# yfukasawa/LongQC

Measured on AMD Instinct MI355X. Metric: Mbases/sec all-vs-all overlap coverage (sampleqc hot path), higher is better.
Workload: dtype u64; 1 GPU; BASELINE configs[2]: 500000 synthetic PacBio Sequel CLR reads ~10 kb 30x, pb-sequel preset (-Y -l 0 -q 160 -k 12 -w 5 -I 4G -p 80), 5000 subsample queries; target_bases=5181693140, query_bases=51577117, parallelism=single GPU

## Files before the change

### longqc_amd/csrc/engine.cpp

```cpp
#include "engine.hpp"
#include "kernels_sketch.hpp"
#include "kernels_index.hpp"
#include "kernels_seed.hpp"
#include "kernels_sort.hpp"
#include "kernels_walk.hpp"
#include "kernels_psort.hpp"
#include "kernels_chain.hpp"
#include "fastx.hpp"
#include "fastx_mem.hpp"
#include "sat_replay.hpp"
#ifndef LQ_EMU
extern "C" void lq_segv_altstack();
#endif
#include <cstdio>
#include <cstring>
#include <cmath>
#include <cinttypes>
#include <algorithm>
#include <unordered_map>
#include <deque>
#include <future>
#include <functional>

static inline u32 nblk(u64 n, u32 bs)
{
	u64 b = (n + bs - 1) / bs;
	if (b > 0x7fffffffULL) throw std::runtime_error("launch too large");
	return (u32)b;
}

template <class T> static void h2d(T *dst, const T *src, size_t n, hipStream_t s)
{
	if (n) LQ_HIP_CHECK(hipMemcpyAsync(dst, src, n * sizeof(T), hipMemcpyHostToDevice, s));
}
template <class T> static void d2h(T *dst, const T *src, size_t n, hipStream_t s)
{
	if (n) { LQ_HIP_CHECK(hipMemcpyAsync(dst, src, n * sizeof(T), hipMemcpyDeviceToHost, s)); LQ_HIP_CHECK(hipStreamSynchronize(s)); }
}
static void dzero(void *p, size_t bytes, hipStream_t s) { if (bytes) LQ_HIP_CHECK(hipMemsetAsync(p, 0, bytes, s)); }
static void check_launch() { LQ_HIP_CHECK(hipGetLastError()); }
static const bool lq_timeline = getenv("LQCOV_TIMELINE") != nullptr;
static double lq_timeline_t0 = 0;
static void lq_tl(const char *who, int id, const char *what, double extra = -1)
{
	if (!lq_timeline) return;
	if (extra >= 0) fprintf(stderr, "[tl] %8.2f %s%d %s %.0f\n", (lq_now_s() - lq_timeline_t0) * 1e3, who, id, what, extra);
	else fprintf(stderr, "[tl] %8.2f %s%d %s\n", (lq_now_s() - lq_timeline_t0) * 1e3, who, id, what);
}
#ifndef LQ_EMU
int lq_trace_launches = 0;
#endif

StageTimer::StageTimer(lqcov_handle *h_, hipStream_t s_, const char *name_, u64 bytes_) : h(h_), s(s_), name(name_), bytes(bytes_)
{
	on = h->profiling && (h->profile_only.empty() || h->profile_only == name_ || ("|" + h->profile_only + "|").find(std::string("|") + name_ + "|") != std::string::npos);
	if (!on) return;
	hipEventCreate(&a); hipEventCreate(&b);
	hipEventRecord(a, s);
}
StageTimer::StageTimer(lqcov_handle *h_, const char *name_, u64 bytes_) : StageTimer(h_, h_->stream, name_, bytes_) {}
StageTimer::~StageTimer()
{
	if (!on) return;
	hipEventRecord(b, s);
	if (h->profiling == 1) { hipEventSynchronize(b); std::lock_guard<std::mutex> g(h->stage_mu); h->account_stage(name, a, b, bytes); }
	else { std::lock_guard<std::mutex> g(h->stage_mu); h->stage_pending.push_back(lqcov_handle::StagePending{name, a, b, bytes}); }
}
void lqcov_handle::account_stage(const char *name, hipEvent_t a, hipEvent_t b, u64 bytes)
{
	float ms = 0; hipEventElapsedTime(&ms, a, b);
	hipEventDestroy(a); hipEventDestroy(b);
	auto it = stages.find(name);
	if (it == stages.end()) { stage_order.push_back(name); it = stages.emplace(name, StageAcc()).first; }
	it->second.ms += ms; it->second.launches += 1; it->second.bytes += bytes;
}
void lqcov_handle::drain_stages()
{
	std::lock_guard<std::mutex> g(stage_mu);
	for (lqcov_handle::StagePending &sp : stage_pending) { hipEventSynchronize(sp.b); account_stage(sp.name, sp.a, sp.b, sp.bytes); }
	stage_pending.clear();
	for (auto &kv : late_bytes) { auto it = stages.find(kv.first); if (it != stages.end()) it->second.bytes += kv.second; }
	late_bytes.clear();
}
void lqcov_handle::add_stage_bytes(const char *name, u64 bytes)
{
	if (!profiling || !bytes) return;
	std::lock_guard<std::mutex> g(stage_mu);
	late_bytes[name] += bytes;
}

void Knobs::read_env()
{
	auto num = [](const char *name, long dflt) { const char *e = getenv(name); return e && *e ? atol(e) : dflt; };
	auto is = [](const char *name, const char *val) { const char *e = getenv(name); return e && !strcmp(e, val); };
	lanes = (int)std::min<long>(8, std::max<long>(1, num("LQCOV_LANES", 3)));
	anchor_budget = getenv("LQCOV_ANCHOR_BUDGET") ? strtoull(getenv("LQCOV_ANCHOR_BUDGET"), 0, 10) : 0;
	query_order_file = is("LQCOV_QUERY_ORDER", "file");
	query_order_striped = is("LQCOV_QUERY_ORDER", "striped");
	all_klib = is("LQCOV_SORT", "klib");
	ps_shift = (u32)std::min<long>(12, std::max<long>(0, num("LQCOV_PS_SHIFT", 0)));
	reg_walker = !is("LQCOV_WALK", "solo");
	ckpt = !is("LQCOV_CKPT", "0");
	ckpt3 = num("LQCOV_CKPT3", 1) > 0;
	sort_tile = (u32)std::max<long>(0, num("LQCOV_SORT_TILE", 0)); if (sort_tile && sort_tile < 64) sort_tile = 64;
	walk_shift = (u32)std::min<long>(16, std::max<long>(0, num("LQCOV_WALK_SHIFT", 0)));
	chain_wave_min = (int)std::max<long>(0, num("LQCOV_CHAIN_WAVE_MIN", 0));
	chain_cap = (int)num("LQCOV_CHAIN_CAP", 128);
	run_stage = (u32)std::max<long>(1, num("LQCOV_RUN_STAGE", LQ_RUN_STAGE));
	run_grid = (u32)std::max<long>(1, num("LQCOV_RUN_GRID", 2048));
	ps_key64 = num("LQCOV_PS_KEY64", 0) != 0;
	sketch_wgen = num("LQCOV_SKETCH_WGEN", 0) != 0;
	upload_amb = num("LQCOV_UPLOAD_AMB", 0) != 0;
	sketch_fast = num("LQCOV_SKETCH_FAST", 1) != 0;
#ifndef LQ_EMU
	lq_trace_launches = (int)num("LQCOV_TRACE_LAUNCHES", 0);
#endif
	no_level_skip = getenv("LQCOV_NO_LEVEL_SKIP") != nullptr;
	debug_sort = getenv("LQCOV_DEBUG_SORT") != nullptr;
	sketch_kpt = (u32)std::min<long>(64, std::max<long>(1, num("LQCOV_SKETCH_KPT", 4)));
	sketch_machine_only = is("LQCOV_SKETCH", "machine");
// ... 568 lines not shown
{
	const u32 n = q.n;
	dzero(lambda.p, (n + 1) * 8, stream); dzero(lambda2.p, (n + 1) * 8, stream);
	dzero(avg_k.p, (n + 1) * 4, stream); dzero(qflags.p, (n + 1) * 4, stream);
	dzero(cnts.p, cnt_count() * 4 + 4, stream);
	dzero(n_pv.p, 4, stream);
	if (!distributed) mid_occ = -1;
	stat_sens_runs = 0; stat_p2_queries = 0; stat_p2_anchors = 0;
	for (auto &v : stat_tie_why) v = 0;
	sat_cnt.clear(); stat_sat_chains = 0; sat_last_valid = false;
	finished = false;
	LQ_HIP_CHECK(hipStreamSynchronize(stream));
	if (lq_timeline) { lq_timeline_t0 = lq_now_s(); lq_tl("main", 0, "reset"); }
}

void lqcov_handle::build_index(Part &pt)
{
	hipStream_t stream = this->bstream; Prim &prim = this->bprim;
	(void)prim;
	ReadSetDev &rs = pt.rs;
	const u64 M = rs.n_mini;
	ix_owner = &pt;
	sat_last_valid = false;
	pt.n_keys = 0; pt.cap_bits = 4;
	pt.pos.ensure(M * 8 + 8);
	std::vector<u32> soff(q.n + 1, 0), srid;
	bool names_done = false;
	auto host_names = [&]() {
		names_done = true;
		if (P.no_self && q.n) {
			std::unordered_map<std::string, std::vector<u32>> byname;
			for (u32 i = 0; i < q.n; ++i) byname[q.names[i]].push_back(i);
			std::vector<std::vector<u32>> per(q.n);
			for (u32 r = 0; r < rs.n; ++r) {
				auto it = byname.find(rs.names[r]);
				if (it != byname.end()) for (u32 qi : it->second) per[qi].push_back(r);
			}
			for (u32 i = 0; i < q.n; ++i) { soff[i + 1] = soff[i] + (u32)per[i].size(); srid.insert(srid.end(), per[i].begin(), per[i].end()); }
		}
		if (P.ava) {
			std::vector<std::string> names(rs.names.begin(), rs.names.end());
			std::sort(names.begin(), names.end());
			names.erase(std::unique(names.begin(), names.end()), names.end());
			std::vector<u32> tr(rs.n + 1, 0), ql(q.n + 1, 0);
			for (u32 r = 0; r < rs.n; ++r) tr[r] = (u32)(std::lower_bound(names.begin(), names.end(), rs.names[r]) - names.begin());
			for (u32 i = 0; i < q.n; ++i) ql[i] = (u32)(std::lower_bound(names.begin(), names.end(), q.names[i]) - names.begin());
			pt.t_rank.ensure((rs.n + 1) * 4); pt.q_lo.ensure((q.n + 1) * 4);
			h2d(pt.t_rank.as<u32>(), tr.data(), rs.n + 1, stream);
			h2d(pt.q_lo.as<u32>(), ql.data(), q.n + 1, stream);
			LQ_HIP_CHECK(hipStreamSynchronize(stream));
		}
	};
	if (M) {
		DBuf &key = ix_key, &key2 = ix_key2, &head = ix_head, &uidx = ix_uidx, &ukey = ix_ukey, &ustart = ix_ustart, &ucnt = ix_ucnt;
		const u64 n_tiles = (M + LQ_HEAD_TILE - 1) / LQ_HEAD_TILE;
		key.ensure(M * 8); key2.ensure(M * 8); head.ensure((n_tiles + 1) * 4); uidx.ensure((n_tiles + 1) * 8);
		const bool k32 = 2 * P.k <= 32;
		const bool fused_heads = 2 * P.k <= 24;
		if (k32) {
			if (!(rs.key_stamp && rs.key_stamp == ix_key_stamp)) { LQ_LAUNCH(k_sort_keys<u32>, nblk(M, 256), 256, stream, rs.mx.as<u64>(), M, key.as<u32>()); check_launch(); }
			ix_key_stamp = 0;
			{ StageTimer t(this, stream, "index_radix_sort", M * 24); prim.sort_pairs_u32_u64(key.as<u32>(), key2.as<u32>(), rs.my.as<u64>(), pt.pos.as<u64>(), M, (unsigned)(2 * P.k), key.as<u32>()); }
			if (!fused_heads) { LQ_LAUNCH(k_head_count<u32>, (u32)n_tiles, LQ_HEAD_THREADS, stream, key2.as<u32>(), M, head.as<u32>()); check_launch(); }
		} else {
			ix_key_stamp = 0;
			LQ_LAUNCH(k_sort_keys<u64>, nblk(M, 256), 256, stream, rs.mx.as<u64>(), M, key.as<u64>()); check_launch();
			{ StageTimer t(this, stream, "index_radix_sort", M * 32); prim.sort_pairs_u64(key.as<u64>(), key2.as<u64>(), rs.my.as<u64>(), pt.pos.as<u64>(), M, (unsigned)(2 * P.k), key.as<u64>()); }
			LQ_LAUNCH(k_head_count<u64>, (u32)n_tiles, LQ_HEAD_THREADS, stream, key2.as<u64>(), M, head.as<u32>()); check_launch();
		}
		u64 K = 0;
		if (fused_heads) {
			const u64 k_max = std::min<u64>(M, (u64)1 << (2 * P.k));
			ukey.ensure(k_max * 8); ustart.ensure(k_max * 8);
			const u64 n_blocks = (n_tiles + LQ_HEADLB_SUB - 1) / LQ_HEADLB_SUB;
			uidx.ensure((n_blocks + 2) * 8 + 64);
			dzero(uidx.p, (n_blocks + 2) * 8 + 64, stream);
			u64 *granules = uidx.as<u64>(), *count = granules + n_blocks; u32 *ticket = (u32*)(granules + n_blocks + 1);
			{
				StageTimer t(this, stream, "k_head_lookback", M * 4);
				LQ_LAUNCH(k_head_lookback<u32>, (u32)n_blocks, LQ_HEAD_THREADS, stream, key2.as<u32>(), M, granules, ticket, ukey.as<u64>(), ustart.as<u64>(), count);
				check_launch();
			}
			host_names();
			d2h(&K, count, 1, stream);
			pt.n_keys = K;
			ucnt.ensure(K * 4);
		} else {
			dzero(head.as<u32>() + n_tiles, 4, stream);
			prim.exclusive_scan_u32_u64(head.as<u32>(), uidx.as<u64>(), n_tiles + 1);
			host_names();
			d2h(&K, uidx.as<u64>() + n_tiles, 1, stream);
			pt.n_keys = K;
			ukey.ensure(K * 8); ustart.ensure(K * 8); ucnt.ensure(K * 4);
			if (k32) LQ_LAUNCH(k_head_fill<u32>, (u32)n_tiles, LQ_HEAD_THREADS, stream, key2.as<u32>(), M, uidx.as<u64>(), ukey.as<u64>(), ustart.as<u64>());
			else LQ_LAUNCH(k_head_fill<u64>, (u32)n_tiles, LQ_HEAD_THREADS, stream, key2.as<u64>(), M, uidx.as<u64>(), ukey.as<u64>(), ustart.as<u64>());
			check_launch();
		}
		LQ_LAUNCH(k_unique_counts, nblk(K, 256), 256, stream, ustart.as<u64>(), K, M, ucnt.as<u32>()); check_launch();
		u32 bits = 4;
		while (((u64)1 << bits) < 2 * K) ++bits;
		pt.cap_bits = bits;
		const u64 cap = (u64)1 << bits;
		pt.tkey.ensure(cap * 8); pt.tstart.ensure(cap * 8); pt.tcnt.ensure(cap * 4);
		LQ_HIP_CHECK(hipMemsetAsync(pt.tkey.p, 0xff, cap * 8, stream));
		{
			StageTimer t(this, stream, "k_table_insert", K * 20 + cap * 8);
			LQ_LAUNCH(k_table_insert, nblk(K, 256), 256, stream, ukey.as<u64>(), ustart.as<u64>(), ucnt.as<u32>(), K, pt.tkey.as<u64>(), pt.tstart.as<u64>(), pt.tcnt.as<u32>(), bits);
			check_launch();
		}
		if (mid_occ <= 0) {
			if (P.mid_occ_frac <= 0.0f) mid_occ = INT32_MAX;
			else {
				DBuf &sorted = ix_sorted; sorted.ensure(K * 4);
				prim.sort_keys_u32(ucnt.as<u32>(), sorted.as<u32>(), K);
				const u32 kth = (u32)((1. - P.mid_occ_frac) * (double)K);
				u32 v = 0;
				d2h(&v, sorted.as<u32>() + kth, 1, stream);
				mid_occ = (i32)(v + 1);
			}
		}
		LQ_HIP_CHECK(hipStreamSynchronize(stream));
	} else {
		const u64 cap = (u64)1 << pt.cap_bits;
		pt.tkey.ensure(cap * 8); pt.tstart.ensure(cap * 8); pt.tcnt.ensure(cap * 4);
		LQ_HIP_CHECK(hipMemsetAsync(pt.tkey.p, 0xff, cap * 8, stream));
		if (mid_occ <= 0) mid_occ = P.mid_occ_frac <= 0.0f ? INT32_MAX : 1;
	}
	if (!names_done) host_names();
	pt.self_off.ensure((q.n + 1) * 4); pt.self_rid.ensure(srid.size() * 4 + 4);
	h2d(pt.self_off.as<u32>(), soff.data(), q.n + 1, stream);
	h2d(pt.self_rid.as<u32>(), srid.data(), srid.size(), stream);
	LQ_HIP_CHECK(hipStreamSynchronize(stream));
	pt.built = true;
	pt.plan.valid = false;
	lq_tl("build", 0, "index done");
	if (K.plan_ahead && have_queries && mid_occ > 0 && !distributed) plan_part(pt, stream, prim);
}

void lqcov_handle::build_part(Part &pt)
{
	if (!have_queries) throw std::logic_error("set the queries before building a part");
	lq_tl("build", 0, "build_part begins (reads uploaded)");
	sketch(pt.rs, true);
	lq_tl("build", 0, "sketched");
	build_index(pt);
	lq_tl("build", 0, "index + seed plan done");
}

static u64 dbg_anchor_sum(const mm128 &a) { u64 h = (a.x * 0x9E3779B97F4A7C15ULL) ^ (a.y * 0xD6E8FEB86659FD93ULL); return h ^ (h >> 29); }

void lqcov_handle::sort_checked(MapLane &L, Part &pt, const u64 *aqb, const u32 *qkb, u32 nqb, u64 a_base, u64 nA, const std::vector<u64> &h_off, const std::vector<u32> &h_klib)
{
	mm128 *dA = L.A.as<mm128>(), *dB = L.B.as<mm128>();
	u64 sum_before = 0;
	if (K.debug_sort) {
		std::vector<mm128> ha(nA), hb(nA);
		d2h(ha.data(), dA, nA, L.stream); d2h(hb.data(), dB, nA, L.stream);
		for (u32 q = 0; q < nqb; ++q)
			for (u64 i = h_off[q]; i < h_off[q + 1]; ++i) sum_before += dbg_anchor_sum(h_klib[q] ? hb[i] : ha[i]);
	}
	sort_batch(L, pt, aqb, qkb, nqb, a_base, nA);
	if (K.debug_sort) {
		std::vector<mm128> ha(nA);
		d2h(ha.data(), dA, nA, L.stream);
		u64 sum_after = 0;
		for (u64 i = 0; i < nA; ++i) sum_after += dbg_anchor_sum(ha[i]);
		if (sum_after != sum_before) fprintf(stderr, "[sort] batch of %u queries: NOT A PERMUTATION of the emitted anchors (sums %016llx / %016llx)\n", nqb, (unsigned long long)sum_before, (unsigned long long)sum_after);
		u64 unsorted = 0, ties = 0, unmarked = 0;
		for (u32 q = 0; q < nqb; ++q)
			for (u64 i = h_off[q] + 1; i < h_off[q + 1]; ++i) {
				if (ha[i].x < ha[i - 1].x) ++unsorted;
				if (ha[i].x == ha[i - 1].x) { ++ties; if (!(ha[i].y & LQ_TIE_MARK) || !(ha[i - 1].y & LQ_TIE_MARK)) { if (unmarked++ < 4) fprintf(stderr, "[sort] query %u of the batch: equal x %016llx, y %016llx / %016llx\n", q, (unsigned long long)ha[i].x, (unsigned long long)ha[i - 1].y, (unsigned long long)ha[i].y); } }
			}
		fprintf(stderr, "[sort] batch of %u queries: %llu anchors, %llu out of order, %llu equal-x neighbours, %llu of them with an unmarked anchor\n", nqb, (unsigned long long)nA, (unsigned long long)unsorted, (unsigned long long)ties, (unsigned long long)unmarked);
// ... 233 lines not shown
		}
	} else if (nj && opt) {
		StageTimer t(this, L.stream, "k_seed_emit", nj * 32 + nA * 24);
		LQ_LAUNCH(k_seed_emit, nblk(nj, LQ_EMIT_THREADS), LQ_EMIT_THREADS, L.stream, q.mx.as<u64>(), q.my.as<u64>(), q_owner.as<u32>(), q.moff.as<u64>(), j0, nj,
		          pt.pos.as<u64>(), hit_start.as<u64>(), hit_n.as<u32>(), keep.as<u32>(), dup.as<u32>(),
		          a_off.as<u64>(), a_base, mp_off.as<u64>(), q.d_len.as<u32>(),
		          (int)P.no_self, pt.self_off.as<u32>(), pt.self_rid.as<u32>(), ava,
		          qzero.as<u32>(), L.A.as<mm128>(), L.B.as<mm128>(), mini_pos.as<u64>(), EmitSub{nullptr, nullptr, nullptr});
		check_launch();
	}
	const u32 ivl_cap = (u32)std::min<u64>(nA / (P.min_cnt > 0 ? P.min_cnt : 1) + 16, 0xfffffff0ULL);
	L.ivl.ensure((u64)ivl_cap * sizeof(Ivl));
	dzero(L.n_ivl.p, 4, L.stream); dzero(L.n_sens.p, 32, L.stream);
	if (nA) {
		const u64 *aqb = (opt ? aqf_off : aq_off).as<u64>() + q0;
		const u32 *qkb = opt ? qzero.as<u32>() : qklib.as<u32>() + q0;
		std::vector<u64> rel; std::vector<u32> hk;
		if (K.debug_sort) {
			rel.resize(nqb + 1); hk.assign(nqb, 0);
			for (u32 i = 0; i <= nqb; ++i) rel[i] = h_off[q0 + i] - a_base;
			if (!opt) d2h(hk.data(), qklib.as<u32>() + q0, nqb, L.stream);
		}
		sort_checked(L, pt, aqb, qkb, nqb, a_base, nA, rel, hk);
		if (opt && !L.gate_passed) { L.gate_passed = true; open_gate(); }
		chain_stage(L, pt, aqb, a_base, nqb, q0, nullptr, nA, opt ? 1 : 0, 0, ivl_cap, dbg);
	}
	u32 n_sens = 0;
	if (nA && opt) {
		u32 ns8[8] = {0};
		d2h(ns8, L.n_sens.as<u32>(), 8, L.stream);
		n_sens = ns8[0];
		for (int i = 1; i <= 6; ++i) stat_tie_why[i - 1] += ns8[i];
	}
	lq_tl("lane", lane_id, "first pass done, anchors", (double)nA);
	if (n_sens) {
		std::vector<u64> want(n_sens);
		d2h(want.data(), L.sens.as<u64>(), n_sens, L.stream);
		std::sort(want.begin(), want.end());
		want.erase(std::unique(want.begin(), want.end()), want.end());
		std::vector<u32> fq;
		for (u64 k : want) if (fq.empty() || fq.back() != (u32)(k >> 32)) fq.push_back((u32)(k >> 32));
		L.want.ensure(want.size() * 8);
		h2d(L.want.as<u64>(), want.data(), want.size(), L.stream);
		LQ_HIP_CHECK(hipStreamSynchronize(L.stream));
		stat_sens_runs += want.size(); stat_p2_queries += fq.size();
		u64 max_mini = 0;
		for (size_t i = 0; i < fq.size(); ) {
			std::vector<u32> sq, sk; std::vector<u64> so{0};
			size_t k = i;
			while (k < fq.size() && (k == i || so.back() + (h_aq[fq[k] + 1] - h_aq[fq[k]]) <= anchor_budget)) {
				const u64 len = h_aq[fq[k] + 1] - h_aq[fq[k]];
				sq.push_back(fq[k]); sk.push_back(len > LQ_RS_MIN ? 1u : 0u); so.push_back(so.back() + len);
				max_mini = std::max<u64>(max_mini, h_qmoff[fq[k] + 1] - h_qmoff[fq[k]]);
				++k;
			}
			stat_p2_anchors += so.back();
			lq_tl("lane", lane_id, "second pass begins, anchors", (double)so.back());
			map_subset(L, pt, sq, sk, so, max_mini, 2, (u32)want.size(), ivl_cap, dbg, nullptr);
			if (lq_timeline) { LQ_HIP_CHECK(hipStreamSynchronize(L.stream)); lq_tl("lane", lane_id, "second pass done"); }
			i = k;
		}
	}
	if (nA) {
		u32 ni = 0;
		d2h(&ni, L.n_ivl.as<u32>(), 1, L.stream);
		if (ni > ivl_cap) throw std::runtime_error("interval pool overflow");
		if (ni) {
			L.iv_q.ensure((u64)ni * 4); L.iv_q2.ensure((u64)ni * 4); L.iv_se.ensure((u64)ni * 8); L.iv_se2.ensure((u64)ni * 8);
			L.ivq_off.ensure((n_q + 1) * 4); L.iv_scratch.ensure((u64)ni * 16);
			LQ_LAUNCH(k_split_ivl, nblk(ni, 256), 256, L.stream, L.ivl.as<Ivl>(), ni, L.iv_q.as<u32>(), L.iv_se.as<u64>()); check_launch();
			L.prim.sort_pairs_u32_u64(L.iv_q.as<u32>(), L.iv_q2.as<u32>(), L.iv_se.as<u64>(), L.iv_se2.as<u64>(), ni, 32);
			LQ_LAUNCH(k_ivl_offsets, nblk(n_q + 1, 256), 256, L.stream, L.iv_q2.as<u32>(), ni, n_q, L.ivq_off.as<u32>()); check_launch();
			std::lock_guard<std::mutex> guard(pv_mu);
			const u64 need = pv_reserved + 2 * (u64)ni;
			if (need > 0xfffffff0ULL) throw std::domain_error("too many persisted intervals");
			if (need > pv_cap) {
				LQ_HIP_CHECK(hipDeviceSynchronize());
				u32 npv = 0;
				d2h(&npv, n_pv.as<u32>(), 1, L.stream);
				grow_keep(pv, (u64)npv * sizeof(Ivl), need * sizeof(Ivl) * 2, L.stream);
				pv_cap = (u32)std::min<u64>(pv.cap / sizeof(Ivl), 0xfffffff0ULL);
			}
			pv_reserved = need;
			StageTimer t(this, L.stream, "k_filter_redundant");
			LQ_LAUNCH(k_filter_redundant, nblk(n_q, 64), 64, L.stream, L.iv_se2.as<u64>(), L.ivq_off.as<u32>(), n_q, (u32)P.min_coverage,
			          L.iv_scratch.as<u32>(), pv.as<Ivl>(), n_pv.as<u32>(), pv_cap);
			check_launch();
		}
	}
}

static PsLists ps_lists(MapLane &L, int set, u32 sh)
{
	PsWork &W = L.ps[set];
	PsLists Ls;
	Ls.big[0] = W.big[0].as<PSeg>(); Ls.big[1] = W.big[1].as<PSeg>(); Ls.fin_s = W.fin_s.as<PSeg>(); Ls.fin_b = W.fin_b.as<PSeg>();
	Ls.cnt = L.sort_cnt.as<u32>() + (set ? LQ_C_PS1 : LQ_C_PS0);
	Ls.cap_big = (u32)std::min<u64>(W.big[0].cap / sizeof(PSeg), 0xfffffff0ULL); Ls.cap_fin = (u32)std::min<u64>(W.fin_s.cap / sizeof(PSeg), 0xfffffff0ULL);
	Ls.fin_s_max = std::max<u32>(LQ_PS_FIN_SMALL >> sh, 2); Ls.fin_b_max = std::max<u32>(LQ_PS_FIN_BIG >> sh, 4); Ls.child_target = std::max<u32>(LQ_PS_CHILD >> sh, 2);
	return Ls;
}

static void ps_pass(lqcov_handle *h, MapLane &L, int set, hipStream_t s, u64 nA, const KeyMap &km, const PsData &pd, u32 cur)
{
	PsWork &W = L.ps[set];
	u32 *cnt = L.sort_cnt.as<u32>() + (set ? LQ_C_PS1 : LQ_C_PS0);
	const PsLists Ls = ps_lists(L, set, h->K.ps_shift);
	const u32 cap_cnt = (u32)std::min<u64>(W.gcnt.cap / 4, 0xfffffff0ULL);
	const u32 g_tiles = (u32)std::min<u64>((nA + LQ_PS_TILE - 1) / LQ_PS_TILE + 1, LQ_PS_GRID);
	const u32 g_segs = (u32)std::min<u64>(Ls.cap_big, 256);
	const u32 nxt = cur ^ 1;
	const u32 cap_tiles = (u32)std::min<u64>(W.tmap.cap / 4, 0xfffffff0ULL);
	LQ_LAUNCH(k_ps_plan, 1, 256, s, Ls.big[cur], cnt + (cur ? LQ_P_BIG1 : LQ_P_BIG0), W.plan.as<PPlan>(), cnt, cap_cnt, cap_tiles, Ls.child_target, cnt + (nxt ? LQ_P_BIG1 : LQ_P_BIG0)); check_launch();
	LQ_LAUNCH(k_ps_tilemap, g_segs, 256, s, W.plan.as<PPlan>(), cnt + (cur ? LQ_P_BIG1 : LQ_P_BIG0), cnt, W.tmap.as<u32>(), cap_tiles, W.gcnt.as<u32>(), W.gdiff.as<unsigned long long>()); check_launch();
	{
		StageTimer t(h, s, "k_ps_hist");
		LQ_LAUNCH(k_ps_hist, g_tiles, LQ_PS_THREADS, s, Ls.big[cur], cnt + (cur ? LQ_P_BIG1 : LQ_P_BIG0), W.plan.as<PPlan>(), W.tmap.as<u32>(), cnt, pd, km, W.gcnt.as<u32>(), W.gdiff.as<unsigned long long>()); check_launch();
	}
	LQ_LAUNCH(k_ps_scan, g_segs, 256, s, Ls.big[cur], cnt + (cur ? LQ_P_BIG1 : LQ_P_BIG0), W.plan.as<PPlan>(), W.gcnt.as<u32>(), W.gcur.as<u32>(), W.gdiff.as<unsigned long long>(), Ls, (u32)(nxt ? LQ_P_BIG1 : LQ_P_BIG0),
	          (unsigned long long*)(L.sort_cnt.as<u32>() + (set ? LQ_C_PART1 : LQ_C_PART0))); check_launch();
	{
		StageTimer t(h, s, "k_ps_scatter");
		LQ_LAUNCH(k_ps_scatter, g_tiles, LQ_PS_THREADS, s, Ls.big[cur], cnt + (cur ? LQ_P_BIG1 : LQ_P_BIG0), W.plan.as<PPlan>(), W.tmap.as<u32>(), cnt, pd, km, W.gcur.as<u32>()); check_launch();
	}
}

static void ps_finish(lqcov_handle *h, MapLane &L, int set, hipStream_t s, u64 nA, const KeyMap &km, const PsData &pd)
{
	u32 *cnt = L.sort_cnt.as<u32>() + (set ? LQ_C_PS1 : LQ_C_PS0);
	const PsLists Ls = ps_lists(L, set, h->K.ps_shift);
	const bool k32 = km.pbits + km.rbits + 1 <= 32 + 8 && !h->K.ps_key64;
	{
		StageTimer t(h, s, "k_ps_finish<8192>");
		unsigned long long *tl = (unsigned long long*)(L.sort_cnt.as<u32>() + (set ? LQ_C_FINB1 : LQ_C_FINB0));
		const u32 g = (u32)std::min<u64>(std::min<u64>(Ls.cap_fin, nA / LQ_PS_FIN_SMALL + 64), LQ_PS_GRID / 4);
		if (!k32) LQ_LAUNCH((k_ps_finish<LQ_PS_FIN_BIG, 1024, 10, u64>), g, 1024, s, Ls.fin_b, cnt + LQ_P_FIN_B, pd, km, tl);
		else LQ_LAUNCH((k_ps_finish<LQ_PS_FIN_BIG, 1024, 10, u32>), g, 1024, s, Ls.fin_b, cnt + LQ_P_FIN_B, pd, km, tl);
		check_launch();
	}
	{
		StageTimer t(h, s, "k_ps_finish<1024>");
		unsigned long long *tl = (unsigned long long*)(L.sort_cnt.as<u32>() + (set ? LQ_C_FINS1 : LQ_C_FINS0));
		const u32 g = (u32)std::min<u64>(std::min<u64>(Ls.cap_fin, nA / 16 + 256), LQ_PS_GRID * 2);
		if (k32) LQ_LAUNCH((k_ps_finish<LQ_PS_FIN_SMALL, 256, 8, u32>), g, 256, s, Ls.fin_s, cnt + LQ_P_FIN_S, pd, km, tl);
		else LQ_LAUNCH((k_ps_finish<LQ_PS_FIN_SMALL, 256, 8, u64>), g, 256, s, Ls.fin_s, cnt + LQ_P_FIN_S, pd, km, tl);
		check_launch();
	}
}


void lqcov_handle::psort_run(MapLane &L, int set, hipStream_t s, u64 nA, const KeyMap &km, const PsData &pd)
{
	u32 *cnt = L.sort_cnt.as<u32>() + (set ? LQ_C_PS1 : LQ_C_PS0);
	if (set == 1) {
		ps_finish(this, L, set, s, nA, km, pd);
		dzero(cnt + LQ_P_FIN_S, 8, s);
	}
	for (u32 pass = 0; pass < K.ps_passes; ++pass) ps_pass(this, L, set, s, nA, km, pd, pass & 1);
	ps_finish(this, L, set, s, nA, km, pd);
}

void lqcov_handle::psort_tail(MapLane &L, int set, hipStream_t s, u64 nA, const KeyMap &km, const PsData &pd)
{
	u32 *cnt = L.sort_cnt.as<u32>() + (set ? LQ_C_PS1 : LQ_C_PS0);
	for (int round = 0; round < 40; ++round) {
		u32 left = 0;
		d2h(&left, cnt + LQ_P_BIG0, 1, s);
		if (!left) return;
		dzero(cnt + LQ_P_FIN_S, 8, s);
		ps_pass(this, L, set, s, nA, km, pd, 0); ps_pass(this, L, set, s, nA, km, pd, 1);
// ... 601 lines not shown
				} catch (...) { errs[li] = std::current_exception(); next.store(batches.size()); gate_cv.notify_all(); }
			});
		for (auto &t : th) t.join();
		for (auto &e : errs) if (e) { hipDeviceSynchronize(); std::rethrow_exception(e); }
	};
	auto cut_batches = [&](const std::vector<u64> &off, u32 g_begin, u32 g_end) {
		std::vector<std::pair<u32, u32>> batches;
		const u64 total = off[g_end] - off[g_begin];
		u64 nb = (total + anchor_budget - 1) / anchor_budget;
		if (nb < (u64)n_lanes && h_aq[g_end] - h_aq[g_begin] >= ((u64)n_lanes << 24)) nb = n_lanes;
		if (nb > (u64)n_lanes) nb = (nb + n_lanes - 1) / n_lanes * n_lanes;
		if (nb == 0) nb = 1;
		u64 left = nb;
		for (u32 q0 = g_begin; q0 < g_end; ) {
			const u64 rem = off[g_end] - off[q0];
			const u64 lim = std::min(anchor_budget, left > 1 ? (rem + left - 1) / left : rem);
			u32 q1 = q0 + 1;
			while (q1 < g_end && off[q1 + 1] - off[q0] <= lim) ++q1;
			batches.emplace_back(q0, q1);
			q0 = q1;
			if (left > 1) --left;
		}
		return batches;
	};
	bool regrouped = false;
	for (u32 g_begin = 0, g_end = n_q; ; ) {
		if (opt && pt.plan.bucketed) { g_begin = pt.plan.q_begin; g_end = pt.plan.q_end; }
		run_batches(cut_batches(opt ? h_aqf : h_aq, g_begin, g_end));
		if (g_end >= n_q) break;
		regrouped = true;
		bool ok = false;
		try { ok = seed_group(pt, pt.plan, true, stream, prim, g_end); }
		catch (const LqOutOfMemory &) { (void)hipGetLastError(); seed_ws.release_large(); ok = false; }
		if (!ok) {
			pt.plan.bucketed = false;
			pt.plan.h_aqf = pt.plan.h_aq;
			LQ_HIP_CHECK(hipMemcpyAsync(aqf_off.p, aq_off.p, (n_q + 1) * 8, hipMemcpyDeviceToDevice, stream));
			LQ_HIP_CHECK(hipStreamSynchronize(stream));
			pt.plan.n_written += h_aq[n_q] - h_aq[g_end];
			g_begin = g_end; g_end = n_q;
		}
		last_n_written = pt.plan.n_written;
	}
	if (regrouped) pt.plan.valid = false;
	if (dbg) { unsigned long long nd = 0; d2h(&nd, n_dbg.as<unsigned long long>(), 1, stream); n_dbg_host = nd; }
	sat_replay_part(pt, h_aq, h_qmoff);
	LQ_HIP_CHECK(hipStreamSynchronize(stream));
	lq_tl("main", 0, "map_part ends");
}

void lqcov_handle::finish()
{
	const u32 n_q = q.n;
	rows.assign(n_q, lqcov_row());
	regs.clear(); mregs.clear();
	if (n_q == 0) { finished = true; return; }
	u32 npv = 0;
	d2h(&npv, n_pv.as<u32>(), 1, stream);
	DBuf rowdev, pvq_off, k1, k2, s1, s2, scratch, dregs, dmregs, cnt2;
	rowdev.ensure((u64)n_q * sizeof(RowDev)); dzero(rowdev.p, (u64)n_q * sizeof(RowDev), stream);
	pvq_off.ensure((n_q + 1) * 4); cnt2.ensure(8); dzero(cnt2.p, 8, stream);
	k1.ensure((u64)npv * 4 + 4); k2.ensure((u64)npv * 4 + 4); s1.ensure((u64)npv * 8 + 8); s2.ensure((u64)npv * 8 + 8);
	scratch.ensure((u64)npv * 8 + 8);
	dregs.ensure(((u64)npv + 1) * sizeof(RegionT)); dmregs.ensure(((u64)npv + 1) * sizeof(RegionT));
	if (npv) {
		LQ_LAUNCH(k_split_ivl, nblk(npv, 256), 256, stream, pv.as<Ivl>(), npv, k1.as<u32>(), s1.as<u64>()); check_launch();
		prim.sort_pairs_u32_u64(k1.as<u32>(), k2.as<u32>(), s1.as<u64>(), s2.as<u64>(), npv, 32);
	}
	LQ_LAUNCH(k_ivl_offsets, nblk(n_q + 1, 256), 256, stream, k2.as<u32>(), npv, n_q, pvq_off.as<u32>()); check_launch();
	{
		StageTimer t(this, "k_reliable");
		LQ_LAUNCH(k_reliable, nblk(n_q, 64), 64, stream, s2.as<u64>(), pvq_off.as<u32>(), n_q, (u32)P.min_coverage, scratch.as<u32>(),
		          dregs.as<RegionT>(), cnt2.as<u32>(), dmregs.as<RegionT>(), cnt2.as<u32>() + 1, rowdev.as<RowDev>());
		check_launch();
	}
	for (auto &kv : sat_cnt) {
		u64 off[2];
		d2h(off, cnt_off_dev() + kv.first, 2, stream);
		if (kv.second.size() != (size_t)(off[1] - off[0])) throw std::logic_error("replayed counters: layout changed");
		h2d(cnts.as<u32>() + off[0], kv.second.data(), kv.second.size(), stream);
	}
	{
		StageTimer t(this, "k_cnt_stats", q.n_mini * 8);
		LQ_LAUNCH(k_cnt_stats, nblk(n_q, 64), 64, stream, cnts.as<u32>(), cnt_off_dev(), own_cnt_layout ? d_nsize.as<u32>() : (const u32*)nullptr, n_q, rowdev.as<RowDev>(), qflags.as<u32>(), cnt_max);
		check_launch();
	}
	std::vector<RowDev> hr(n_q);
	std::vector<u64> hl(n_q), hl2(n_q), hmoff(n_q + 1);
	std::vector<float> hk(n_q);
	std::vector<u32> hf(n_q);
	std::vector<double> hp(n_q);
	u32 nr[2] = {0, 0};
	d2h(hr.data(), rowdev.as<RowDev>(), n_q, stream);
	d2h(hl.data(), lambda.as<u64>(), n_q, stream); d2h(hl2.data(), lambda2.as<u64>(), n_q, stream);
	d2h(hk.data(), avg_k.as<float>(), n_q, stream); d2h(hf.data(), qflags.as<u32>(), n_q, stream);
	d2h(hp.data(), qual_psum.as<double>(), n_q, stream);
	d2h(hmoff.data(), q.moff.as<u64>(), n_q + 1, stream);
	d2h(nr, cnt2.as<u32>(), 2, stream);
	regs.resize(nr[0]); mregs.resize(nr[1]);
	static_assert(sizeof(RegionT) == sizeof(lqcov_region), "region layout");
	d2h((RegionT*)regs.data(), dregs.as<RegionT>(), nr[0], stream);
	d2h((RegionT*)mregs.data(), dmregs.as<RegionT>(), nr[1], stream);
	for (u32 i = 0; i < n_q; ++i)
		if (hf[i] & 2u)
			throw std::domain_error("query " + q.names[i] + ": a chain matched a minimizer beyond the counters sized from the command line's -k/-w/-H; "
			                        "the reference overruns its counter array there (minimap2-coverage.c:422, esterr.c:131) -- pass the prebuilt index's -k/-w/-H");
	for (u32 i = 0; i < n_q; ++i) {
		lqcov_row &r = rows[q_perm[i]];
		r.lambda = hl[i]; r.lambda2 = hl2[i]; r.qual_psum = hp[i]; r.qlen = q.h_len[i];
		r.n_mini = own_cnt_layout ? h_nsize[i] : (u32)(hmoff[i + 1] - hmoff[i]); r.n_match = hr[i].n_match; r.avg_k = hk[i];
		r.reg_off = hr[i].reg_off; r.n_reg = hr[i].n_reg; r.mreg_off = hr[i].mreg_off; r.n_mreg = hr[i].n_mreg;
		r.has_qual = q_has_qual ? 1u : 0u; r.flags = hf[i] | (sat_cnt.count(i) ? LQCOV_ROW_REPLAYED : 0u);
	}
	finished = true;
}

void lq_format_rows(FILE *out, int filter_flag, const lqcov_row *rows, u32 n_rows, const lqcov_region *regs, const lqcov_region *mregs,
                    const std::function<const char *(u32)> &name_of)
{
	std::string line;
	char buf[128];
	for (u32 i = 0; i < n_rows; ++i) {
		const lqcov_row &r = rows[i];
		const double div = r.n_match > 0 ? logf((float)r.n_mini / (float)(int32_t)r.n_match) / r.avg_k : 1.0;
		double mq;
		if (r.has_qual) mq = -10 * log10(r.qual_psum / (int)r.qlen);
		else { volatile double z = 0.0; volatile int zl = 0; mq = -10 * log10(z / zl); }
		line.clear();
		line += name_of(i); line += '\t';
		snprintf(buf, sizeof(buf), "%d\t%" PRIu64 "\t", (int)r.qlen, r.lambda); line += buf;
		if (r.n_reg > 0) {
			u32 tot = 0;
			for (u32 k = 0; k < r.n_reg; ++k) {
				const lqcov_region &g = regs[r.reg_off + k];
				snprintf(buf, sizeof(buf), "%s%d-%d", k ? "," : "", (int)g.start, (int)g.end); line += buf;
				tot += g.end - g.start;
			}
			line += '\t';
			if (r.n_mreg > 0) {
				for (u32 k = 0; k < r.n_mreg; ++k) {
					const lqcov_region &g = mregs[r.mreg_off + k];
					snprintf(buf, sizeof(buf), "%s%d-%d", k ? "," : "", (int)g.start, (int)g.end); line += buf;
				}
			} else line += '0';
			if (filter_flag) snprintf(buf, sizeof(buf), "\t%.3f\t%.3f\t%.3f\t0.0\n", (double)tot / (int)r.qlen, mq, div);
			else snprintf(buf, sizeof(buf), "\t%.3f\t%.3f\t%.3f\t%.3f\n", (double)r.lambda / tot, mq, div, (double)r.lambda2 / tot);
			line += buf;
		} else {
			snprintf(buf, sizeof(buf), "0\t0\t0.0\t%.3f\t%.3f\t0.0\n", mq, div); line += buf;
		}
		fwrite(line.data(), 1, line.size(), out);
	}
}

void lqcov_handle::write_table(FILE *out)
{
	if (!finished) throw std::logic_error("finish() has not run");
	lq_format_rows(out, P.filter_flag, rows.data(), q.n, regs.data(), mregs.data(), [&](u32 i) { return q.names[q_inv[i]].c_str(); });
}

void lqcov_handle::write_table_set(u32 set, FILE *out)
{
	if (!finished) throw std::logic_error("finish() has not run");
	if (set + 1 >= set_first.size()) throw std::invalid_argument("no such query set");
	const u32 a = set_first[set];
	lq_format_rows(out, P.filter_flag, rows.data() + a, set_first[set + 1] - a, regs.data(), mregs.data(), [&](u32 i) { return q.names[q_inv[a + i]].c_str(); });
}

#define LQ_MMI_MAGIC "MMI\2"
#define LQ_MMI_BUCKET_BITS 14
#define LQ_MMI_NO_SEQ 0x2

static void fwrite_or_throw(const void *p, size_t sz, size_t n, FILE *fp)
{
	if (n && fwrite(p, sz, n, fp) != n) throw std::runtime_error("write to the index dump failed");
}

void lqcov_handle::adopt_index_params(i32 k, i32 w, i32 hpc)
{
	if (k == P.k && w == P.w && (hpc != 0) == (P.hpc != 0)) return;
	if (k < 1 || k > 28 || w < 1 || w > 255) throw std::domain_error("prebuilt index with k or w outside [1,28] / [1,255]");
	if (!parts.empty()) for (auto &p : parts) if (p && p->live) throw std::logic_error("index parameters change with live parts");
	std::vector<u64> old(q.n + 1, 0);
	if (have_queries && q.n) d2h(old.data(), q.moff.as<u64>(), q.n + 1, stream);
	P.k = k; P.w = w; P.hpc = hpc ? 1 : 0;
// ... 454 lines not shown
```

### longqc_amd/csrc/kernels_chain.hpp

```cpp
#pragma once
#include "lq_common.hpp"
#include "kernels_sketch.hpp"
#include "kernels_sort.hpp"

#define LQ_RUN_TILE 4096
#define LQ_RUN_THREADS 256
#define LQ_RUN_ROWS (LQ_RUN_TILE / LQ_RUN_THREADS)
#define LQ_RUN_WAVES (LQ_RUN_THREADS / 64)

#define LQ_TSCAN_THREADS 1024
__global__ void __launch_bounds__(LQ_TSCAN_THREADS)
k_tile_scan(u32 *cnt, u32 n)
{
	__shared__ u32 wsum[LQ_TSCAN_THREADS / 64];
	const u32 t = threadIdx.x, lane = t & 63, w = t >> 6;
	const u32 per = (n + LQ_TSCAN_THREADS - 1) / LQ_TSCAN_THREADS;
	const u32 a = (u64)t * per < n ? t * per : n, b = a + per < n ? a + per : n;
	u32 sum = 0;
	for (u32 x = a; x < b; ++x) sum += cnt[x];
	u32 inc = sum;
	for (int d = 1; d < 64; d <<= 1) { const u32 o = __shfl_up(inc, d); if ((int)lane >= d) inc += o; }
	if (lane == 63) wsum[w] = inc;
	__syncthreads();
	if (t == 0) { u32 run = 0; for (u32 x = 0; x < LQ_TSCAN_THREADS / 64; ++x) { const u32 v = wsum[x]; wsum[x] = run; run += v; } cnt[n] = run; }
// ... 973 lines not shown
		if (e & 2) {
			if (e & 1) { if (e & 4) med_cov -= min_cov; else --med_cov; }
			else       { if (e & 4) med_cov += min_cov; else ++med_cov; }
		}
		if (old < min_cov && med_cov >= min_cov) med_start = e;
		else if (old >= min_cov && med_cov < min_cov) {
			const u32 mlen = (e >> 3) - med_start;
			if (mlen > 0) {
				mc[2 * n_mc] = med_start; mc[2 * n_mc + 1] = e; ++n_mc;
				u32 s = atomicAdd(n_pv, 1u);
				if (s < pv_cap) { Ivl m; m.q = q; m.start = med_start | 4u; m.end = e | 4u; pv[s] = m; }
			}
		}
	}
	for (u32 i = 0; i < n; ++i) {
		const u32 s0 = (u32)cv[i], e0 = (u32)(cv[i] >> 32);
		bool inside = false;
		for (u32 j = 0; j < n_mc; ++j) if (s0 >= mc[2 * j] && e0 <= mc[2 * j + 1]) { inside = true; break; }
		if (!inside) {
			u32 s = atomicAdd(n_pv, 1u);
			if (s < pv_cap) { Ivl m; m.q = q; m.start = s0; m.end = e0; pv[s] = m; }
		}
	}
}

__global__ void k_split_ivl(const Ivl *iv, u32 n, u32 *qkey, u64 *se)
{
	u32 i = blockIdx.x * blockDim.x + threadIdx.x;
	if (i >= n) return;
	qkey[i] = iv[i].q; se[i] = (u64)iv[i].start | (u64)iv[i].end << 32;
}

struct RegionT { u32 start, end; };

template <bool WRITE>
__device__ __forceinline__ void lq_sweep(const u32 *vc, u32 n2, u32 min_cov, RegionT *regs, RegionT *mregs, u32 &n_reg, u32 &n_mreg)
{
	u32 start = 0, cov = 0, med_start = 0, med_cov = 0;
	n_reg = n_mreg = 0;
	for (u32 j = 0; j < n2; ++j) {
		const u32 e = vc[j], old_cov = cov, old_med = med_cov;
		if (e & 1) {
			--cov;
			if (e & 2) { if (e & 4) { med_cov -= min_cov; cov -= (min_cov - 1); } else --med_cov; }
		} else {
			++cov;
			if (e & 2) { if (e & 4) { med_cov += min_cov; cov += (min_cov - 1); } else ++med_cov; }
		}
		if (old_cov < min_cov && cov >= min_cov) {
			start = e >> 3;
			if (old_med < min_cov && med_cov >= min_cov) med_start = e >> 3;
		} else if (old_cov >= min_cov && cov < min_cov) {
			if ((e >> 3) - start > 0) { if (WRITE) { regs[n_reg].start = start; regs[n_reg].end = e >> 3; } ++n_reg; }
			if (old_med >= min_cov && med_cov < min_cov)
				if ((e >> 3) - med_start > 0) { if (WRITE) { mregs[n_mreg].start = med_start; mregs[n_mreg].end = e >> 3; } ++n_mreg; }
		} else if (old_med < min_cov && med_cov >= min_cov) {
			med_start = e >> 3;
		} else if (old_med >= min_cov && med_cov < min_cov) {
			if ((e >> 3) - med_start > 0) { if (WRITE) { mregs[n_mreg].start = med_start; mregs[n_mreg].end = e >> 3; } ++n_mreg; }
		}
	}
}

struct RowDev {
	u32 n_match, reg_off, n_reg, mreg_off, n_mreg;
};

__global__ void k_reliable(const u64 *se, const u32 *pvq_off, u32 n_q, u32 min_cov, u32 *scratch ,
                           RegionT *regs, u32 *n_regs, RegionT *mregs, u32 *n_mregs, RowDev *rows)
{
	u32 q = blockIdx.x * blockDim.x + threadIdx.x;
	if (q >= n_q) return;
	const u32 lo = pvq_off[q], n = pvq_off[q + 1] - lo;
	u32 *vc = scratch + (u64)lo * 2;
	for (u32 i = 0; i < n; ++i) { vc[2 * i] = (u32)se[lo + i]; vc[2 * i + 1] = (u32)(se[lo + i] >> 32); }
	lq_heapsort_u32(vc, 2 * (i64)n);
	u32 nr, nm;
	lq_sweep<false>(vc, 2 * n, min_cov, nullptr, nullptr, nr, nm);
	u32 ro = nr ? atomicAdd(n_regs, nr) : 0, mo = nm ? atomicAdd(n_mregs, nm) : 0;
	lq_sweep<true>(vc, 2 * n, min_cov, regs + ro, mregs + mo, nr, nm);
	rows[q].reg_off = ro; rows[q].n_reg = nr; rows[q].mreg_off = mo; rows[q].n_mreg = nm;
}

__global__ void k_cnt_stats(const u32 *cnts, const u64 *cnt_off, const u32 *nsize, u32 n_q, RowDev *rows, u32 *qflags, u32 cnt_max)
{
	u32 q = blockIdx.x * blockDim.x + threadIdx.x;
	if (q >= n_q) return;
	const u64 lo = cnt_off[q], hi = nsize ? lo + nsize[q] : cnt_off[q + 1];
	u32 sum = 0, n = (u32)(hi - lo), nm = 0;
	bool sat = false;
	for (u64 j = lo; j < hi; ++j) { sum += cnts[j] & cnt_max; if (cnts[j] >= cnt_max) sat = true; }
	if (sat) atomicOr(&qflags[q], 1u);
	if (nsize) {
		bool over = false;
		for (u64 j = hi; j < cnt_off[q + 1]; ++j) if (cnts[j]) over = true;
		if (over) atomicOr(&qflags[q], 2u);
	}
	if (n) sum /= n;
	for (u64 j = lo; j < hi; ++j) if ((cnts[j] & cnt_max) > sum) ++nm;
	rows[q].n_match = nm;
}

__global__ void k_qual_sum(const u8 *qual, const u64 *seq_off, u32 n_q, const double *q2p, double *psum)
{
	u32 q = blockIdx.x * blockDim.x + threadIdx.x;
	if (q >= n_q) return;
	double s = 0.0;
	for (u64 i = seq_off[q]; i < seq_off[q + 1]; ++i) {
		int v = (int)(signed char)qual[i] - 33;
		v = v < 0 ? 0 : v > 126 ? 126 : v;
		s += q2p[v];
	}
	psum[q] = s;
}
```

Baseline: 15220 Mbases/s.

## Parallelize k_cnt_stats per wavefront and batch result D2H copies

```diff
diff --git a/longqc_amd/csrc/engine.cpp b/longqc_amd/csrc/engine.cpp
--- a/longqc_amd/csrc/engine.cpp
+++ b/longqc_amd/csrc/engine.cpp
@@ -36,6 +36,10 @@
 template <class T> static void d2h(T *dst, const T *src, size_t n, hipStream_t s)
 {
 	if (n) { LQ_HIP_CHECK(hipMemcpyAsync(dst, src, n * sizeof(T), hipMemcpyDeviceToHost, s)); LQ_HIP_CHECK(hipStreamSynchronize(s)); }
+}
+template <class T> static void d2h_queue(T *dst, const T *src, size_t n, hipStream_t s)
+{
+	if (n) LQ_HIP_CHECK(hipMemcpyAsync(dst, src, n * sizeof(T), hipMemcpyDeviceToHost, s));
 }
 static void dzero(void *p, size_t bytes, hipStream_t s) { if (bytes) LQ_HIP_CHECK(hipMemsetAsync(p, 0, bytes, s)); }
 static void check_launch() { LQ_HIP_CHECK(hipGetLastError()); }
@@ -770,14 +774,18 @@
 				check_launch();
 			}
 			host_names();
+			lq_tl("build", 0, "  host_names done");
 			d2h(&K, count, 1, stream);
+			lq_tl("build", 0, "  sort + run heads waited for");
 			pt.n_keys = K;
 			ucnt.ensure(K * 4);
 		} else {
 			dzero(head.as<u32>() + n_tiles, 4, stream);
 			prim.exclusive_scan_u32_u64(head.as<u32>(), uidx.as<u64>(), n_tiles + 1);
 			host_names();
+			lq_tl("build", 0, "  host_names done");
 			d2h(&K, uidx.as<u64>() + n_tiles, 1, stream);
+			lq_tl("build", 0, "  sort + run heads waited for");
 			pt.n_keys = K;
 			ukey.ensure(K * 8); ustart.ensure(K * 8); ucnt.ensure(K * 4);
 			if (k32) LQ_LAUNCH(k_head_fill<u32>, (u32)n_tiles, LQ_HEAD_THREADS, stream, key2.as<u32>(), M, uidx.as<u64>(), ukey.as<u64>(), ustart.as<u64>());
@@ -1177,10 +1185,12 @@
 				pv_cap = (u32)std::min<u64>(pv.cap / sizeof(Ivl), 0xfffffff0ULL);
 			}
 			pv_reserved = need;
+			if (lq_timeline) { LQ_HIP_CHECK(hipStreamSynchronize(L.stream)); lq_tl("lane", lane_id, "  intervals sorted"); }
 			StageTimer t(this, L.stream, "k_filter_redundant");
 			LQ_LAUNCH(k_filter_redundant, nblk(n_q, 64), 64, L.stream, L.iv_se2.as<u64>(), L.ivq_off.as<u32>(), n_q, (u32)P.min_coverage,
 			          L.iv_scratch.as<u32>(), pv.as<Ivl>(), n_pv.as<u32>(), pv_cap);
 			check_launch();
+			if (lq_timeline) { LQ_HIP_CHECK(hipStreamSynchronize(L.stream)); lq_tl("lane", lane_id, "  k_filter_redundant done"); }
 		}
 	}
 }
@@ -1948,7 +1958,7 @@
 	}
 	{
 		StageTimer t(this, "k_cnt_stats", q.n_mini * 8);
-		LQ_LAUNCH(k_cnt_stats, nblk(n_q, 64), 64, stream, cnts.as<u32>(), cnt_off_dev(), own_cnt_layout ? d_nsize.as<u32>() : (const u32*)nullptr, n_q, rowdev.as<RowDev>(), qflags.as<u32>(), cnt_max);
+		LQ_LAUNCH(k_cnt_stats, nblk(n_q, LQ_CS_THREADS / 64), LQ_CS_THREADS, stream, cnts.as<u32>(), cnt_off_dev(), own_cnt_layout ? d_nsize.as<u32>() : (const u32*)nullptr, n_q, rowdev.as<RowDev>(), qflags.as<u32>(), cnt_max);
 		check_launch();
 	}
 	std::vector<RowDev> hr(n_q);
@@ -1957,16 +1967,17 @@
 	std::vector<u32> hf(n_q);
 	std::vector<double> hp(n_q);
 	u32 nr[2] = {0, 0};
-	d2h(hr.data(), rowdev.as<RowDev>(), n_q, stream);
-	d2h(hl.data(), lambda.as<u64>(), n_q, stream); d2h(hl2.data(), lambda2.as<u64>(), n_q, stream);
-	d2h(hk.data(), avg_k.as<float>(), n_q, stream); d2h(hf.data(), qflags.as<u32>(), n_q, stream);
-	d2h(hp.data(), qual_psum.as<double>(), n_q, stream);
-	d2h(hmoff.data(), q.moff.as<u64>(), n_q + 1, stream);
+	d2h_queue(hr.data(), rowdev.as<RowDev>(), n_q, stream);
+	d2h_queue(hl.data(), lambda.as<u64>(), n_q, stream); d2h_queue(hl2.data(), lambda2.as<u64>(), n_q, stream);
+	d2h_queue(hk.data(), avg_k.as<float>(), n_q, stream); d2h_queue(hf.data(), qflags.as<u32>(), n_q, stream);
+	d2h_queue(hp.data(), qual_psum.as<double>(), n_q, stream);
+	d2h_queue(hmoff.data(), q.moff.as<u64>(), n_q + 1, stream);
 	d2h(nr, cnt2.as<u32>(), 2, stream);
 	regs.resize(nr[0]); mregs.resize(nr[1]);
 	static_assert(sizeof(RegionT) == sizeof(lqcov_region), "region layout");
-	d2h((RegionT*)regs.data(), dregs.as<RegionT>(), nr[0], stream);
-	d2h((RegionT*)mregs.data(), dmregs.as<RegionT>(), nr[1], stream);
+	d2h_queue((RegionT*)regs.data(), dregs.as<RegionT>(), nr[0], stream);
+	d2h_queue((RegionT*)mregs.data(), dmregs.as<RegionT>(), nr[1], stream);
+	LQ_HIP_CHECK(hipStreamSynchronize(stream));
 	for (u32 i = 0; i < n_q; ++i)
 		if (hf[i] & 2u)
 			throw std::domain_error("query " + q.names[i] + ": a chain matched a minimizer beyond the counters sized from the command line's -k/-w/-H; "
diff --git a/longqc_amd/csrc/kernels_chain.hpp b/longqc_amd/csrc/kernels_chain.hpp
--- a/longqc_amd/csrc/kernels_chain.hpp
+++ b/longqc_amd/csrc/kernels_chain.hpp
@@ -1079,23 +1079,27 @@
 	rows[q].reg_off = ro; rows[q].n_reg = nr; rows[q].mreg_off = mo; rows[q].n_mreg = nm;
 }
 
-__global__ void k_cnt_stats(const u32 *cnts, const u64 *cnt_off, const u32 *nsize, u32 n_q, RowDev *rows, u32 *qflags, u32 cnt_max)
-{
-	u32 q = blockIdx.x * blockDim.x + threadIdx.x;
+#define LQ_CS_THREADS 256
+__global__ void __launch_bounds__(LQ_CS_THREADS)
+k_cnt_stats(const u32 *cnts, const u64 *cnt_off, const u32 *nsize, u32 n_q, RowDev *rows, u32 *qflags, u32 cnt_max)
+{
+	const u32 lane = threadIdx.x & 63;
+	const u32 q = blockIdx.x * (LQ_CS_THREADS / 64) + threadIdx.x / 64;
 	if (q >= n_q) return;
-	const u64 lo = cnt_off[q], hi = nsize ? lo + nsize[q] : cnt_off[q + 1];
-	u32 sum = 0, n = (u32)(hi - lo), nm = 0;
-	bool sat = false;
-	for (u64 j = lo; j < hi; ++j) { sum += cnts[j] & cnt_max; if (cnts[j] >= cnt_max) sat = true; }
-	if (sat) atomicOr(&qflags[q], 1u);
-	if (nsize) {
-		bool over = false;
-		for (u64 j = hi; j < cnt_off[q + 1]; ++j) if (cnts[j]) over = true;
-		if (over) atomicOr(&qflags[q], 2u);
-	}
+	const u64 lo = cnt_off[q], end = cnt_off[q + 1], hi = nsize ? lo + nsize[q] : end;
+	const u32 n = (u32)(hi - lo);
+	u32 sum = 0, flg = 0, nm = 0;
+	for (u64 j = lo + lane; j < hi; j += 64) { const u32 c = cnts[j]; sum += c & cnt_max; if (c >= cnt_max) flg |= 1u; }
+	if (nsize)
+		for (u64 j = hi + lane; j < end; j += 64) if (cnts[j]) flg |= 2u;
+	for (int o = 32; o > 0; o >>= 1) { sum += __shfl_xor(sum, o); flg |= __shfl_xor(flg, o); }
 	if (n) sum /= n;
-	for (u64 j = lo; j < hi; ++j) if ((cnts[j] & cnt_max) > sum) ++nm;
-	rows[q].n_match = nm;
+	for (u64 j = lo + lane; j < hi; j += 64) if ((cnts[j] & cnt_max) > sum) ++nm;
+	for (int o = 32; o > 0; o >>= 1) nm += __shfl_xor(nm, o);
+	if (lane == 0) {
+		if (flg) atomicOr(&qflags[q], flg);
+		rows[q].n_match = nm;
+	}
 }
 
 __global__ void k_qual_sum(const u8 *qual, const u64 *seq_off, u32 n_q, const double *q2p, double *psum)
```

Result: no change. 15190 Mbases/s (-0.2%).
